# tool-recommender-bot/logparser

Measured on AMD Instinct MI355X. Metric: GB/s (and lines/s) of 'combined' log parsed per GPU and per 8xMI355X node, higher is better.
Workload: dtype u8

## Files before the change

logparser_amd/csrc/lp_device.h:

```cpp
#pragma once
#include <cstddef>
#include <type_traits>
#include <utility>

#include "lp_program.h"
#include "lp_fixed.h"

namespace lp {

enum : int { ST_OK = 0, ST_BAD = 1, ST_FALLBACK = 2,
             ST_REDO = 3,
             ST_REPAIR = 4 };

#if defined(LP_PROFILE) && defined(__HIP__)
static __device__ unsigned long long g_prof[PROF_WAVES * PROF_POINTS];
#endif
#if defined(LP_PROFILE) && defined(__HIP_DEVICE_COMPILE__)
__device__ __forceinline__ void lp_prof_mark(int k) {
    const unsigned long long t = clock64();
    const unsigned w = blockIdx.x - PROF_W0;
    const uint64_t act = __ballot(1);
    if (w < (unsigned)PROF_WAVES && (int)threadIdx.x % 64 == (int)__builtin_ctzll(act))
        __builtin_nontemporal_store(t, &g_prof[w * PROF_POINTS + k]);
}
// ... 2692 lines not shown

template <typename BP>
__host__ __device__ LP_INLINE bool utf8_ok(BP b, uint32_t n) {
    for (uint32_t i = 0; i < n;) {
        uint32_t c = b[i];
        if (c < 0x80) { ++i; continue; }
        int need;
        uint32_t cp;
        if (c >= 0xC2 && c <= 0xDF) { need = 1; cp = c & 0x1F; }
        else if (c >= 0xE0 && c <= 0xEF) { need = 2; cp = c & 0x0F; }
        else if (c >= 0xF0 && c <= 0xF4) { need = 3; cp = c & 0x07; }
        else return false;
        if (i + (uint32_t)need >= n) return false;
        for (int r = 1; r <= need; ++r) {
            if ((b[i + r] & 0xC0) != 0x80) return false;
            cp = (cp << 6) | (b[i + r] & 0x3F);
        }
        if (need == 2 && (cp < 0x800 || (cp >= 0xD800 && cp <= 0xDFFF))) return false;
        if (need == 3 && (cp < 0x10000 || cp > 0x10FFFF)) return false;
        i += need + 1;
    }
    return true;
}

template <typename LN>
__host__ __device__ LP_INLINE uint64_t decode_span(const LN& L, int a, int b, Arena& A) {
    uint32_t start = A.used;
    for (int q = a; q < b;) {
        uint32_t c = L[q];
        if (c == '%') { A.put(hexv(L[q + 1]) * 16 + hexv(L[q + 2])); q += 3; }
        else { A.put(c); ++q; }
    }
    if (!utf8_ok(A.p + start, A.used - start)) return ~0ull;
    return mkref(start, A.used - start, true);
}

__host__ __device__ LP_INLINE void put_encoded(Arena& A, uint32_t c) {
    const char* HX = "0123456789ABCDEF";
    A.put('%');
    A.put(HX[c >> 4]);
    A.put(HX[c & 15]);
}

__host__ __device__ LP_INLINE void store_word(LP_G uint8_t* p, uint32_t v) {
#if defined(__HIP_DEVICE_COMPILE__)
    *reinterpret_cast<LP_G uint32_t*>(p) = v;
#else
    __builtin_memcpy(p, &v, 4);
#endif
}
template <typename LN>
__host__ __device__ LP_INLINE uint64_t url_decode_value(const LN& L, int vs, int e, Arena& A) {
    const uint32_t st = A.used;
    uint32_t W = (L.o + (uint32_t)vs) >> 2;
    uint64_t ww = (uint64_t)L.word(W) | ((uint64_t)L.word_or0(W + 1) << 32);
    uint64_t acc = 0;
    uint32_t na = 0, out = st;
    for (int q = vs; q < e;) {
        while (na < 4 && q < e) {
            const uint32_t k = L.o + (uint32_t)q - 4 * W;
            const uint32_t c = (uint32_t)(ww >> (8 * k)) & 0xFFu;
            if (c == '%') {
                const uint32_t v =
                    hexv((uint32_t)(ww >> (8 * k + 8)) & 0xFFu) * 16 + hexv((uint32_t)(ww >> (8 * k + 16)) & 0xFFu);
                if (v < 0x80) { acc |= (uint64_t)v << (8 * na); na += 1; }
                else { acc |= (uint64_t)((0xC0 | (v >> 6)) | ((0x80 | (v & 0x3F)) << 8)) << (8 * na); na += 2; }
                q += 3;
            } else {
                acc |= (uint64_t)(c == '+' ? ' ' : c) << (8 * na);
                na += 1;
                ++q;
            }
            if (L.o + (uint32_t)q >= 4 * (W + 1)) {
                ++W;
                ww = (ww >> 32) | ((uint64_t)L.word_or0(W + 1) << 32);
            }
        }
        store_word(A.p + out, (uint32_t)acc);
        if (na >= 4) { out += 4; na -= 4; acc >>= 32; }
        else { out += na; na = 0; acc = 0; }
    }
    if (na) { store_word(A.p + out, (uint32_t)acc); out += na; }
    A.used = out;
    return mkref(st, A.used - st, true);
}

constexpr uint64_t REF_SKIP = ~0ull;

struct QueryTable {
    uint32_t tab = 0, reg = 0, count = 0, maxp = 0;
    int s = 0;
    int lp = -1;
    bool on = false, set = false;
    __host__ __device__ LP_INLINE void emit(LP_G uint8_t* region, int e) {
        if (e > s) {
            const uint64_t t0 = (uint64_t)(uint32_t)s | ((uint64_t)(uint32_t)e << 16) | ((uint64_t)(uint32_t)(lp + 1) << 48);
#if defined(__HIP_DEVICE_COMPILE__)
            typedef uint32_t u32x4_t __attribute__((ext_vector_type(4)));
            *reinterpret_cast<LP_G u32x4_t*>(region + tab + 16 * count) = u32x4_t{(uint32_t)t0, (uint32_t)(t0 >> 32), 0u, 0u};
#else
            LP_G uint64_t* t = (LP_G uint64_t*)(region + tab) + 2 * count;
            t[0] = t0;
            t[1] = 0;
#endif
            ++count;
        }
        lp = -1;
    }
};

template <typename LN>
__host__ __device__ LP_INLINE int piece_eq_rw(const LN& L, int s, int e, bool& rw) {
    rw = false;
    if (s >= e) return -1;
    const uint32_t A = L.o + (uint32_t)s, E = L.o + (uint32_t)e;
    uint32_t W = A >> 2;
    uint32_t valid = swar::HI << (8 * (A & 3));
    for (;;) {
        const uint32_t w = L.word(W);
        const uint32_t r = E - 4 * W;
        if (r < 4) valid &= swar::HI >> (8 * (4 - r));
        const uint32_t meq = swar::eq(w, '=') & valid;
        const uint32_t mrw = (swar::upper(w) | swar::needs_encode(w)) & valid;
        if (meq) {
            rw = rw || (mrw & ((meq & (0u - meq)) - 1u)) != 0;
            return (int)(4 * W + (uint32_t)swar::first(meq) - L.o);
        }
        rw = rw || mrw != 0;
        ++W;
        if (4 * W >= E) return -1;
        valid = swar::HI;
    }
}

struct QPrep {
    int s = 0, e = 0, eq = -1;
    bool rw = false, pv = false;
    uint32_t need = 0;
};
template <typename LN>
__host__ __device__ LP_INLINE QPrep query_prep(const LN& L, uint64_t t0) {
    QPrep q;
    q.s = (int)(t0 & 0xFFFFu);
    q.e = (int)((t0 >> 16) & 0xFFFFu);
    const int lp = (int)((t0 >> 48) & 0xFFFFu) - 1;
    q.eq = piece_eq_rw(L, q.s, q.e, q.rw);
    q.pv = q.eq >= 0 && lp > q.eq;
    const int ne = q.eq >= 0 ? q.eq : q.e;
    q.need = (q.rw ? (3u * (uint32_t)(ne - q.s) + 3u) & ~3u : 0u) + (q.pv ? ((uint32_t)(q.e - q.eq - 1) + 3u) & ~3u : 0u);
    return q;
}

template <typename LN>
__host__ __device__ LP_INLINE uint32_t query_finish(const Program& P, const QueryStage& Q, const LN& L, Arena& A,
                                                    const LP_G uint8_t* region, LP_G uint64_t* slot, const QPrep& qp) {
    const int s = qp.s, e = qp.e, eq = qp.eq;
    const int ne = eq >= 0 ? eq : e;
    const uint32_t a1 = A.used;
    uint64_t nref;
    if (qp.rw) {
        const char* HX = "0123456789abcdef";
        const uint32_t mark = A.used;
        for (int q = s; q < ne; ++q) {
            const uint32_t c = L[q];
            if (uri_needs_encode(c)) { A.put('%'); A.put(HX[c >> 4]); A.put(HX[c & 15]); }
            else A.put((c - 'A') < 26u ? (c | 32) : c);
        }
        nref = mkref(mark, A.used - mark, true);
        A.used = (A.used + 3) & ~3u;
    } else {
        nref = src_ref(L, s, ne - s);
    }
    bool want = Q.want_all;
    const uint32_t nlen = ref_len(nref);
    for (int k = 0; k < Q.n_names && !want; ++k) {
        if (Q.name_len[k] != nlen) continue;
        bool same = true;
        for (uint32_t q = 0; q < nlen && same; ++q) {
            const uint32_t c = qp.rw ? (uint32_t)region[ref_off(nref) + q] : L[s + (int)q];
            same = c == P.lit_byte((int)(Q.name_off[k] + q));
        }
        want = same;
    }
    if (!want) {
        slot[0] = REF_SKIP;
        slot[1] = 0;
        return A.used - a1;
    }
    uint64_t vref;
    if (eq < 0) vref = mkref(0, 0, false);
    else if (!qp.pv) vref = src_ref(L, eq + 1, e - eq - 1);
    else vref = url_decode_value(L, eq + 1, e, A);
    slot[0] = nref;
    slot[1] = vref;
    return A.used - a1;
}

template <typename LN>
__host__ __device__ LP_INLINE uint32_t query_piece(const Program& P, const QueryStage& Q, const LN& L, Arena& R,
                                                   LP_G uint64_t* slot) {
    const QPrep qp = query_prep(L, slot[0]);
    Arena A;
    if (!spill(R, qp.need, A)) {
        slot[0] = REF_SKIP;
        slot[1] = 0;
        return 0;
    }
    return query_finish(P, Q, L, A, R.p, slot, qp);
}

struct UriWalk {
    int fa = -1, h = -1, nh = 0, first_pct = -1;
    uint32_t rewr = 0;
    int resume = -1;
    QueryTable T;
};

template <typename LN>
__host__ __device__ LP_INLINE void uri_walk_fast(const Program& P, int u, const LN& L, int a, int b, uint32_t usep,
                                                 Arena& A, UriWalk& Wk) {
    const UriStage& U = P.uri[u];
    const int qsi = U.want_query ? U.query_stage : -1;
    QueryTable& T = Wk.T;
    int& fa = Wk.fa;
    int& first_pct = Wk.first_pct;
    uint32_t& rewr = Wk.rewr;
    int& resume = Wk.resume;
    LP_PROF(50 + 4 * u);
    for_uev_w(L, a, b, [&](int q, uint32_t w) {
        const uint32_t c = w & 0xFFu;
        if (c == '#' || c == ';' || c >= 0x80) { resume = q; return false; }
        if (c == '%') {
            if (q + 2 >= b || !is_hex((w >> 8) & 0xFFu) || !is_hex((w >> 16) & 0xFFu)) { resume = q; return false; }
            first_pct = first_pct < 0 ? q : first_pct;
            T.lp = q;
            return true;
        }
        if (c == '&' || c == '?') {
            rewr |= (c == '?' && fa >= 0) ? 2u : 0u;
            if (T.on) {
                T.emit(A.p, q);
                T.s = q + 1;
            } else if (fa < 0 && qsi >= 0) {
                T.on = T.set = true;
                T.maxp = usep + 1;
                T.tab = (A.used + 15) & ~15u;
                T.reg = T.tab + 16 * T.maxp;
                T.s = q + 1;
            }
            fa = fa < 0 ? q : fa;
            return true;
        }
        rewr |= (fa >= 0 && uri_needs_encode(c)) ? 2u : 0u;
        T.lp = c == '+' ? q : T.lp;
        return true;
    });
    LP_PROF(51 + 4 * u);
}

enum : int { UR_OFF = 0, UR_ON = 1, UR_DONE = 2 };
template <typename LN, typename Cols>
__host__ __device__ LP_INLINE int uri_repair(const Program& P, int u, const LN& L, int a, int b, Arena& R, Cols& C,
                                             int64_t li);

template <int MODE = UR_ON, typename LN, typename Cols, typename UO>
__host__ __device__ LP_INLINE int uri_stage_rest(const Program& P, int u, const LN& L, int a, int b, uint32_t usep,
                                                 Arena& A, Cols& C, int64_t li, UO& o, UriWalk& Wk,
                                                 int rfa = -1, bool noamp = false) {
    const UriStage& U = P.uri[u];
    const int qsi = U.want_query ? U.query_stage : -1;
    QueryTable& T = Wk.T;
    int& fa = Wk.fa;
    int& h = Wk.h;
    int& nh = Wk.nh;
    int& first_pct = Wk.first_pct;
    uint32_t& rewr = Wk.rewr;
    const int resume = Wk.resume;
    int st = ST_OK;
    if (resume >= 0) for_uev(L, resume, b, [&](int q, uint32_t c) {
        if (c >= 0x80) { st = ST_FALLBACK; return false; }
        if (c == '%') {
            if constexpr (MODE != UR_DONE)
                if (q + 2 >= b || !is_hex(L[q + 1]) || !is_hex(L[q + 2])) { st = ST_REPAIR; return false; }
            if (first_pct < 0) first_pct = q;
            rewr |= h >= 0 ? 1u : 0u;
            if (T.on && h < 0) T.lp = q;
        } else if (c == '#') {
            ++nh;
            if (T.on && h < 0) {
                T.emit(A.p, q);
                T.on = false;
            }
            if (h < 0) h = q;
            if constexpr (MODE != UR_DONE) {
                if (q + 1 < b) {
                    const uint32_t d = L[q + 1];
                    if (d == '&' || d == '?' || d == 'x') { st = ST_REPAIR; return false; }
                }
                if (q > a && L[q - 1] == '=') { st = ST_REPAIR; return false; }
            }
        } else if (c == ';') {
            if constexpr (MODE != UR_DONE) {
                int r = q - 1;
                while (r >= a && (is_alnum(L[r]) || L[r] == '#')) --r;
                if (r >= a && (L[r] == '&' || L[r] == '?')) { st = ST_REPAIR; return false; }
            }
        } else if ((c == '&' || c == '?')) {
            rewr |= (c == '?' && fa >= 0 && h < 0) ? 2u : 0u;
            if (T.on) {
                T.emit(A.p, q);
                T.s = q + 1;
            } else if (fa < 0 && h < 0 && qsi >= 0) {
                T.on = T.set = true;
                T.maxp = usep + 1;
                T.tab = (A.used + 15) & ~15u;
                T.reg = T.tab + 16 * T.maxp;
                T.s = q + 1;
            }
            if (fa < 0) fa = q;
            rewr |= h >= 0 ? 1u : 0u;
        } else {
            const bool enc = uri_needs_encode(c);
            rewr |= (fa >= 0 && h < 0 && enc) ? 2u : 0u;
            if (T.on && c == '+') T.lp = q;
        }
        return true;
    });
    LP_PROF(52 + 4 * u);
    bool fix = false;
    if constexpr (MODE == UR_ON) fix = st == ST_REPAIR;
    if (st != ST_OK && !fix) return st;
    if (!fix && T.set) {
        if (T.on) T.emit(A.p, b);
        A.used = T.reg;
        A.slack += 16 * (T.maxp - T.count);
        C.q_count[qsi][li] = T.count;
        C.q_params[qsi][li] = mkref(T.tab, 16 * T.count, true);
        o.qlist.set(qsi, T.tab);
        o.qpend.set(qsi, T.count);
    }
    LP_PROF(30 + 8 * u);
    if constexpr (MODE == UR_OFF) {
        if (nh > 1) return ST_REPAIR;
    } else if constexpr (MODE == UR_ON) {
        if (!fix && nh > 1) {
// ... 631 lines not shown
```

logparser_amd/csrc/uri.hip:

```cpp
#include "kernels_common.h"

namespace lp {

namespace {

constexpr uint32_t URI_CAP = 8512;
#ifndef LP_URI_QR
#define LP_URI_QR 4
#endif
#ifndef LP_URI_GR
#define LP_URI_GR 9
#endif

constexpr int OWNER_WORDS = LP_URI_GR;
constexpr int OWNER_LDS_WORDS = OWNER_WORDS + PW / 2;
struct OwnerRounds {
    uint64_t* hw;
    uint32_t* tab;
    uint32_t first;
    bool has;
    uint32_t b0;

    __device__ __forceinline__ OwnerRounds(uint64_t* words, uint32_t first_item, uint32_t cnt)
        : hw(words), tab(reinterpret_cast<uint32_t*>(words + OWNER_WORDS)), first(first_item), has(cnt != 0), b0(0) {
// ... 34 lines not shown
template <int NU>
__device__ __forceinline__ UriLane<NU> uri_lane(const Program& P, const Columns& C, int64_t li, bool active) {
    UriLane<NU> U;
    U.sp.fill(0);
    U.cs.fill(0);
    U.usep.fill(0);
    U.ok = false;
    U.fmt = 0;
    U.ls = 0;
    if (!active) return U;
    const uint8_t st = C.status[li];
    const int fmt = P.n_fmt > 1 ? (int)C.fmt_id[li] : 0;
    U.ls = C.line_off[li];
    const uint32_t tf = C.tok_flags[li];
    uint32_t raw[NU], kind[NU];
    for (int u = 0; u < NU; ++u) {
        raw[u] = 0;
        kind[u] = FL_FULL;
        if (u >= P.n_uri || P.uri[u].src_q >= 0) continue;
        if (P.uri[u].src_tok >= 0) {
            raw[u] = C.tok_span[P.uri[u].src_tok][li];
            kind[u] = (tf >> P.uri[u].src_tok) & 1u ? FL_NONE : FL_FULL;
        } else {
            raw[u] = C.fl_uri[P.uri[u].src_fl][li];
            kind[u] = C.fl_kind[P.uri[u].src_fl][li];
        }
    }
    U.ok = st == ST_OK;
    U.fmt = U.ok ? fmt : 0;
    if (U.ok)
        for (int u = 0; u < P.n_uri && u < NU; ++u) {
            const int a = (int)(raw[u] & 0xFFFF), b = (int)(raw[u] >> 16);
            if (P.uri[u].fmt == U.fmt && P.uri[u].src_q < 0 && kind[u] != FL_NONE && b > a) U.sp.set(u, mkspan(a, b));
        }
    return U;
}


template <bool SLOT, typename CL>
__device__ __forceinline__ void uri_walk_coop(const Program& P, int u, const CL& L, bool part, int a, int b,
                                              uint32_t usep, const Arena& A, uint64_t* heads, UriWalk& Wk) {
    const int lane = lane_id();
    const bool table = u >= 0 && P.uri[u].want_query && P.uri[u].query_stage >= 0;
    const uint32_t cnt = part ? usep : 0u;
    const uint32_t x = wave_incl_scan_dpp(cnt);
    const uint32_t eb = x - cnt, E = lane_value(x, 63);
    OwnerRounds OW(heads, eb, cnt);
    const uint32_t tab = (A.used + 15) & ~15u;
    const unsigned long long reg = (unsigned long long)(uintptr_t)A.p;
    int resume = -1, fa = -1, fpct = -1, lastB = -1, lastPP = -1;
    uint32_t count = 0;
    bool rw = false;
    for (uint32_t g0 = 0; g0 < E; g0 += PW) {
        const uint32_t g = g0 + (uint32_t)lane;
        const bool valid = g < E;
        OW.fill_at(g0);
        uint32_t ebo;
        const int ow = OW.owner(g0, ebo);
        const uint32_t oo = (uint32_t)__shfl((int)L.o, ow);
        const int oa = __shfl(a, ow), ob = __shfl(b, ow);
        uint32_t Aq = 0;
        if (valid) {
            const uint32_t A0 = oo + (uint32_t)oa, A1 = oo + (uint32_t)ob, WL = (A1 - 1) >> 6;
            uint32_t W = A0 >> 6, k = g - ebo;
            uint64_t m = L.mask(MC_UEV, W) & (~0ull << (A0 & 63));
            for (;;) {
                if (W == WL) m &= ~0ull >> (63 - ((A1 - 1) & 63));
                const uint32_t c = (uint32_t)__popcll(m);
                if (k < c || W >= WL) break;
                k -= c;
                ++W;
                m = L.mask(MC_UEV, W);
            }
            Aq = (W << 6) + select64(m, k);
        }
        const int q = (int)(Aq - oo);
        CL Lo = L;
        Lo.o = oo;
        Lo.n = ob;
        const uint32_t w = valid ? load_u32_at(Lo, q) : 0u;
        const uint32_t c = w & 0xFFu;
        const bool pct = c == '%';
        const bool bad_pct = pct && (q + 2 >= ob || !is_hex((w >> 8) & 0xFFu) || !is_hex((w >> 16) & 0xFFu));
        const bool stop = valid && (c == '#' || c == ';' || c >= 0x80 || bad_pct);
        const bool aq = c == '&' || c == '?';
        const int cres = __shfl(resume, ow), cfa = __shfl(fa, ow), clB = __shfl(lastB, ow), clPP = __shfl(lastPP, ow);
        const uint32_t ccount = (uint32_t)__shfl((int)count, ow);
        const int s0 = (int)ebo - (int)g0;
        const uint64_t below = (1ull << lane) - 1ull;
        const uint64_t seg_lt = valid ? below & (~0ull << (s0 > 0 ? s0 : 0)) : 0ull;
        const uint64_t Bstop = __ballot(stop);
        const bool live = valid && !stop && cres < 0 && !(Bstop & seg_lt);
        const uint64_t Baq = __ballot(live && aq);
        const uint64_t mfa = Baq & seg_lt;
        const int qfa = __shfl(q, mfa ? lsb64(mfa) : lane);
        const int fa_j = cfa >= 0 ? cfa : (mfa ? qfa : -1);
        const bool pp = live && ((pct && !bad_pct) || c == '+');
        const bool otable = SLOT ? __shfl((int)table, ow) != 0 : table;
        const bool isB = otable && live && aq && fa_j >= 0;
        const uint64_t BB = __ballot(isB), BPP = __ballot(pp);
        const uint64_t mB = BB & seg_lt, mP = BPP & seg_lt;
        const int qpb = __shfl(q, mB ? msb64(mB) : lane), qpp = __shfl(q, mP ? msb64(mP) : lane);
        const bool first_piece = !mB && clB < 0;
        const int pb = mB ? qpb : (clB >= 0 ? clB : fa_j);
        const int lpp = mP ? qpp : clPP;
        const int lp = first_piece ? lpp : (lpp > pb ? lpp : -1);
        const bool emit = isB && q > pb + 1;
        const uint64_t BE = __ballot(emit);
        const bool rwj = live && fa_j >= 0 && ((aq && c == '?') || (!aq && !pct && uri_needs_encode(c)));
        const uint64_t BR = __ballot(rwj);
        const unsigned long long oreg = __shfl(reg, ow);
        const uint32_t otab = (uint32_t)__shfl((int)tab, ow);
        if (emit) {
            const uint32_t idx = ccount + (uint32_t)__popcll(BE & seg_lt);
            const uint64_t t0 = (uint64_t)(uint32_t)(pb + 1) | ((uint64_t)(uint32_t)q << 16) | ((uint64_t)(uint32_t)(lp + 1) << 48);
            *reinterpret_cast<LP_G u32x4*>(reinterpret_cast<LP_G uint8_t*>(oreg) + otab + 16 * idx) =
                u32x4{(uint32_t)t0, (uint32_t)(t0 >> 32), 0u, 0u};
        }
        const int so = (int)eb - (int)g0, eo = (int)(eb + cnt) - (int)g0;
        const int so_c = so < 0 ? 0 : so > PW ? PW : so, eo_c = eo < 0 ? 0 : eo > PW ? PW : eo;
        const uint64_t segm = so_c < eo_c ? ((eo_c == PW ? ~0ull : (1ull << eo_c) - 1ull) & (~0ull << so_c)) : 0ull;
        const uint64_t ms = Bstop & segm, mf = Baq & segm, mpct = __ballot(live && pct) & segm, mb = BB & segm,
                       mpp = BPP & segm;
        const int q_s = __shfl(q, ms ? lsb64(ms) : lane), q_f = __shfl(q, mf ? lsb64(mf) : lane);
        const int q_p = __shfl(q, mpct ? lsb64(mpct) : lane), q_b = __shfl(q, mb ? msb64(mb) : lane);
        const int q_pp = __shfl(q, mpp ? msb64(mpp) : lane);
        if (resume < 0 && ms) resume = q_s;
        if (fa < 0 && mf) fa = q_f;
        if (fpct < 0 && mpct) fpct = q_p;
        if (mb) lastB = q_b;
        if (mpp) lastPP = q_pp;
        count += (uint32_t)__popcll(BE & segm);
        rw = rw || (BR & segm) != 0;
    }
    if (!part) return;
    Wk.resume = resume;
    Wk.fa = fa;
    Wk.first_pct = fpct;
    Wk.rewr = rw ? 2u : 0u;
    QueryTable& T = Wk.T;
    if (table && fa >= 0) {
        T.on = T.set = true;
        T.maxp = usep + 1;
        T.tab = tab;
        T.reg = tab + 16 * T.maxp;
        T.s = (lastB >= 0 ? lastB : fa) + 1;
        T.count = count;
        T.lp = lastB >= 0 ? (lastPP > lastB ? lastPP : -1) : lastPP;
    } else {
        T.lp = lastPP;
    }
}

template <int NU, int NQ, bool COOP, bool SLOT, bool QUEUE, typename LU, typename LL>
__device__ __forceinline__ void uri_wave(const Program& P, const Columns& C, UriLane<NU>& U, LU&& lu, LL&& ll,
                                         bool active, int64_t li, int64_t wave, uint64_t* heads, WaveCounts& WC,
                                         bool& redo) {
    const int lane = lane_id();
    const int nq = P.n_query < NQ ? P.n_query : NQ;
    uint32_t need = 0;
    if (U.ok)
        for (int u = 0; u < P.n_uri && u < NU; ++u) {
            const uint32_t s = U.sp.get(u);
            if (!s) continue;
            uint32_t ev;
            need += uri_need(P, u, lu(u), (int)(s & 0xFFFF), (int)(s >> 16), ev);
            U.usep.set(u, ev);
        }
    int lend = 0;
    if (U.ok) {
        for (int j = 0; j < P.n_list; ++j)
            if (P.list[j].fmt == U.fmt) lend = max(lend, (int)(C.tok_span[P.list[j].tok][li] >> 16));
        for (int j = 0; j < P.n_pair; ++j)
            if (P.pair[j].fmt == U.fmt) lend = max(lend, (int)(C.tok_span[P.pair[j].tok][li] >> 16));
    }
    if (lend) ll(lend, [&](const auto& LH) { need += list_need(P, U.fmt, LH, C, li) + pair_need(P, U.fmt, LH, C, li); });
    need = (need + 15) & ~15u;
    LP_PROF(29);
    const uint32_t x = wave_incl_scan_dpp(need);
    const uint32_t total = lane_value(x, 63);
    LP_PROF(20);
    const int shard = (int)(wave % ARENA_SHARDS);
    unsigned long long wbase = 0;
    if (lane == 63 && total) wbase = atomicAdd(&C.meta->shard_top[16 * shard], (unsigned long long)total + 12ull);
    wbase = (__shfl(wbase, 63) + 15) & ~15ull;
    const bool fits = wbase + total <= C.shard_cap;
    LP_PROF(26);
    uint32_t written = 0;
    unsigned long long my_region = 0;
    UriOutT<NQ> o;
    o.qlist.fill(0);
    o.qpend.fill(0);
    o.status = U.ok ? ST_OK : ST_BAD;
    Arena A{C.arena, 0, 0};
    bool live = false;
    if (U.ok) {
        if (!fits && need) {
            o.status = ST_FALLBACK;
            atomicAdd(&C.meta->arena_ovf, 1ull);
        } else {
            const unsigned long long mine = (unsigned long long)shard * C.shard_cap + wbase + x - need;
            my_region = mine;
            C.arena_base[li] = mine;
            A = Arena{C.arena + mine, 0, need};
            A.top = &C.meta->shard_top[16 * shard];
            A.base = wbase + x - need;
            A.limit = C.shard_cap;
            live = true;
        }
    }
    const int nu = P.n_uri < NU ? P.n_uri : NU;
    for (int sl = 0; sl < nu; ++sl) {
        int u = sl;
        if constexpr (SLOT) {
            u = -1;
            for (int v = 0, c = 0; v < nu; ++v)
                if (P.uri[v].fmt == U.fmt) {
                    if (c == sl) u = v;
                    ++c;
                }
            if (!__any(u >= 0)) break;
        }
        const bool fmt_ok = live && o.status == ST_OK && u >= 0 && P.uri[u].fmt == U.fmt;
        const uint32_t sp = U.sp.get(u);
        const int a = (int)(sp & 0xFFFF), b = (int)(sp >> 16);
        const bool part = fmt_ok && b > a;
        if (fmt_ok && !part) {
            C.u_flags[u][li] = 0;
            if (P.uri[u].query_stage >= 0) { C.q_count[P.uri[u].query_stage][li] = 0; C.q_params[P.uri[u].query_stage][li] = 0; }
        }
        LP_PROF(10 + 2 * sl);
        UriWalk Wk;
        if constexpr (COOP) {
            LP_PROF(50 + 4 * sl);
            uri_walk_coop<SLOT>(P, u, lu(u), part, a, b, U.usep.get(u), A, heads, Wk);
            LP_PROF(51 + 4 * sl);
        } else if (part) {
            uri_walk_fast(P, u, lu(u), a, b, U.usep.get(u), A, Wk);
        }
        if (part) {
            const int st = uri_stage_rest<UR_OFF>(P, u, lu(u), a, b, U.usep.get(u), A, C, li, o, Wk);
            if (st != ST_OK) o.status = st;
        }
        LP_PROF(11 + 2 * sl);
    }
    if (live && lend && o.status == ST_OK) {
        bool filled = true;
        ll(lend, [&](const auto& LH) { filled = list_fill(P, U.fmt, LH, A, C, li) && pair_fill(P, U.fmt, LH, A, C, li); });
        if (!filled) o.status = ST_FALLBACK;
    }
    if (live) {
        if (A.ovf) {
            o.status = ST_FALLBACK;
            atomicAdd(&C.meta->arena_ovf, 1ull);
        }
        written = A.used - A.slack + A.extra;
    }
    LP_PROF(21);
    if (nq > 0) {
        constexpr int QR = LP_URI_QR;
        __syncthreads();
        const bool has = U.ok && o.status == ST_OK && need != 0;
        const unsigned long long my_ab = has ? my_region : 0ull;
        uint64_t piece_ovf = 0;
        uint32_t np = 0;
        for (int qs = 0; qs < nq; ++qs) np += has ? o.qpend.get(qs) : 0u;
        const uint32_t incl = wave_incl_scan_dpp(np);
        const uint32_t base = incl - np, tot = lane_value(incl, 63);
        OwnerRounds OW(heads, base, np);
        auto piece = [&](int ow, uint32_t j, int& pq, uint32_t& soff) {
            uint32_t cum = 0;
            pq = 0;
            soff = 0;
            for (int qs = 0; qs < nq; ++qs) {
                const uint32_t c = (uint32_t)__shfl((int)(has ? o.qpend.get(qs) : 0u), ow);
                const uint32_t l = (uint32_t)__shfl((int)o.qlist.get(qs), ow);
                if (j >= cum && j < cum + c) {
                    pq = qs;
                    soff = l + 16 * (j - cum);
                }
                cum += c;
            }
        };
        auto owner_view = [&](int ow, int pq) {
            auto OL = owner_line(lu(P.query[0].uri), ow);
            for (int qs = 1; qs < nq; ++qs) {
                const auto V = owner_line(lu(P.query[qs].uri), ow);
                if (pq == qs) OL = V;
            }
            return OL;
        };
        for (uint32_t g0 = 0; g0 < tot; g0 += QR * PW) {
            int own[QR], pqs[QR];
            uint32_t soffs[QR];
            uint64_t t0[QR];
#pragma unroll
            for (int k = 0; k < QR; ++k) {
                own[k] = 0;
                pqs[k] = 0;
                soffs[k] = 0;
                t0[k] = 0;
                if (g0 + (uint32_t)(k * PW) >= tot) continue;
                const uint32_t g = g0 + (uint32_t)(k * PW + lane);
                OW.fill_at(g0 + (uint32_t)(k * PW));
                uint32_t ob;
                const int ow = OW.owner(g0 + (uint32_t)(k * PW), ob);
                own[k] = ow;
                const unsigned long long oab = __shfl(my_ab, ow);
                piece(ow, g - ob, pqs[k], soffs[k]);
                if (g < tot) t0[k] = *reinterpret_cast<const LP_G uint64_t*>(C.arena + oab + soffs[k]);
            }
            LP_PROF(17);
            QPrep qp[QR];
            uint32_t mine = 0;
#pragma unroll
            for (int k = 0; k < QR; ++k) {
                if (g0 + (uint32_t)(k * PW) >= tot) continue;
                const uint32_t g = g0 + (uint32_t)(k * PW + lane);
                const auto OL = owner_view(own[k], pqs[k]);
                if (g < tot) qp[k] = query_prep(OL, t0[k]);
                mine += qp[k].need;
            }
            LP_PROF(18);
            const uint32_t x = wave_incl_scan_dpp(mine);
            const uint32_t rtot = lane_value(x, 63);
            unsigned long long rbase = 0;
            if (lane == 63 && rtot) rbase = atomicAdd(&C.meta->shard_top[16 * shard], (unsigned long long)rtot);
            unsigned long long at = __shfl(rbase, 63) + x - mine;
            LP_PROF(19);
#pragma unroll
            for (int k = 0; k < QR; ++k) {
                if (g0 + (uint32_t)(k * PW) >= tot) continue;
                const uint32_t g = g0 + (uint32_t)(k * PW + lane);
                const int ow = own[k];
                const unsigned long long oab = __shfl(my_ab, ow);
                const auto OL = owner_view(ow, pqs[k]);
                bool povf = false;
                if (g < tot) {
                    LP_G uint64_t* slot = reinterpret_cast<LP_G uint64_t*>(C.arena + oab + soffs[k]);
                    const unsigned long long rel = oab - (unsigned long long)shard * C.shard_cap;
                    if (qp[k].need && (at + qp[k].need > C.shard_cap || at - rel + qp[k].need > 0x7FFFFFFFull)) {
                        slot[0] = REF_SKIP;
                        slot[1] = 0;
                        povf = true;
                        atomicAdd(&C.meta->arena_ovf, 1ull);
                    } else {
                        Arena A{C.arena + oab, (uint32_t)(at - rel), (uint32_t)(at - rel + qp[k].need)};
                        written += query_finish(P, P.query[pqs[k]], OL, A, C.arena + oab, slot, qp[k]);
                    }
                    at += qp[k].need;
                }
                for (uint64_t m = __ballot(povf); m; m &= m - 1) piece_ovf |= 1ull << __shfl(ow, (int)__builtin_ctzll(m));
            }
        }
        if (((piece_ovf >> lane) & 1) && o.status == ST_OK) o.status = ST_FALLBACK;
    }
    LP_PROF(22);
    redo = false;
    if (U.ok && o.status == ST_REPAIR) {
        o.status = ST_FALLBACK;
        if constexpr (QUEUE) {
            const unsigned long long k = atomicAdd(&C.meta->uri_fix_lines, 1ull);
            if (k < (unsigned long long)C.cap_lines) C.uri_fix_list[k] = (uint32_t)li;
        } else {
            redo = true;
        }
    }
    if (U.ok && o.status != ST_OK) C.status[li] = (uint8_t)o.status;
    for (int d = 32; d > 0; d >>= 1) written += __shfl_xor(written, d);
    const int st = !active ? -1 : U.ok ? o.status : (int)C.status[li];
    WC.act += (uint32_t)__popcll(__ballot(active));
    WC.ok += (uint32_t)__popcll(__ballot(st == ST_OK));
    WC.bad += (uint32_t)__popcll(__ballot(st == ST_BAD));
    WC.written += written;
}


template <int NU, int NQ, bool SLOT, uint32_t CAP>
__device__ __forceinline__ bool uri_compact(const uint8_t* __restrict__ buf, uint64_t nbytes, const Program& P,
                                            const Columns& C, int64_t wave, int64_t n_lines, uint32_t* cbuf,
                                            uint64_t* plane, uint64_t* heads, WaveCounts& WC, bool& redo) {
    const int lane = lane_id();
    const int64_t li = wave * PW + lane;
    const bool active = li < n_lines;
    LP_PROF(23);
    UriLane<NU> U = uri_lane<NU>(P, C, li, active);
    LP_PROF(27);
    uint64_t lo = ~0ull, hi = 0;
    for (int u = 0; u < P.n_uri && u < NU; ++u) {
        const uint32_t s = U.sp.get(u);
        if (!s) continue;
        lo = min(lo, U.ls + (s & 0xFFFF));
        hi = max(hi, U.ls + (s >> 16));
    }
    const uint64_t r0 = hi ? lo & ~15ull : 0;
    const uint32_t nb1 = hi ? (uint32_t)((((hi + 15) & ~15ull) - r0) >> 4) : 0u;
    const bool lists = P.n_list > 0 || P.n_pair > 0;
    uint64_t l0 = ~0ull, l1 = 0;
    if (lists && U.ok) {
        auto add = [&](int tok) {
            const uint32_t s = C.tok_span[tok][li];
            if ((s >> 16) > (s & 0xFFFFu)) {
                l0 = min(l0, U.ls + (s & 0xFFFFu));
                l1 = max(l1, U.ls + (s >> 16));
            }
        };
        for (int j = 0; j < P.n_list; ++j)
            if (P.list[j].fmt == U.fmt) add(P.list[j].tok);
        for (int j = 0; j < P.n_pair; ++j)
            if (P.pair[j].fmt == U.fmt) add(P.pair[j].tok);
    }
    const uint64_t q0 = l1 ? l0 & ~15ull : 0;
    const uint32_t nb2 = l1 ? (uint32_t)((((l1 + 15) & ~15ull) - q0) >> 4) : 0u;
    auto blocks = [&](uint32_t n, uint32_t& first) {
        const uint32_t x = wave_incl_scan_dpp(n);
        first = x - n;
        return lane_value(x, 63);
    };
    uint32_t cb, nb = nb1 + nb2;
    uint32_t tot = blocks(nb, cb);
    bool lin = lists;
    if (lists && 16 * tot + 16 > CAP) {
        lin = false;
        nb = nb1;
        tot = blocks(nb, cb);
    }
    if (16 * tot + 16 > CAP) return false;
    WC.gathered = 16 * tot;
    for (int u = 0; u < P.n_uri && u < NU; ++u) {
        const uint32_t s = U.sp.get(u);
        if (s) U.cs.set(u, 16 * cb + (uint32_t)(U.ls + (s & 0xFFFF) - r0));
    }
    constexpr int GR = LP_URI_GR;
    uint16_t* pl16 = reinterpret_cast<uint16_t*>(plane);
    OwnerRounds OW(heads, cb, nb);
    for (uint32_t g0 = 0; g0 < tot; g0 += GR * PW) {
        u32x4 v[GR];
        OW.fill(g0);
#pragma unroll
        for (int k = 0; k < GR; ++k) {
            v[k] = u32x4{0, 0, 0, 0};
            if (g0 + (uint32_t)(k * PW) >= tot) continue;
            const uint32_t g = g0 + (uint32_t)(k * PW + lane);
            uint32_t ocb;
            const int own = OW.owner(g0 + (uint32_t)(k * PW), ocb);
            const uint32_t j = g - ocb;
            uint64_t src = (uint64_t)__shfl((unsigned long long)r0, own) + 16ull * j;
            if (lin) {
                const uint32_t n1 = (uint32_t)__shfl(nb1, own);
                const uint64_t s1 = (uint64_t)__shfl((unsigned long long)q0, own);
                if (j >= n1) src = s1 + 16ull * (j - n1);
            }
            if (g < tot) v[k] = load16(buf, nbytes, src);
        }
        LP_PROF(28);
#pragma unroll
        for (int k = 0; k < GR; ++k) {
            const uint32_t g = g0 + (uint32_t)(k * PW + lane);
            if (g >= tot) continue;
            *reinterpret_cast<u32x4*>(cbuf + 4 * g) = v[k];
            pl16[g] = (uint16_t)bcls::classify16u(v[k][0], v[k][1], v[k][2], v[k][3]);
        }
    }
    LP_PROF(24);
    for (uint32_t g = tot + lane; g < ((tot + 1 + 3) & ~3u); g += PW) {
        *reinterpret_cast<u32x4*>(cbuf + 4 * g) = u32x4{0, 0, 0, 0};
        pl16[g] = 0;
    }
    __syncthreads();
    LP_PROF(25);
    typedef LineT<lds_bytes, lds_u64, 1> CL;
    auto lu = [&](int u) {
        const uint32_t s = U.sp.get(u);
        return CL{(lds_bytes)cbuf, U.cs.get(u) - (s & 0xFFFFu), (int)(s >> 16), (lds_u64)plane};
    };
    const LP_G uint8_t* lsp = (const LP_G uint8_t*)buf + U.ls;
    const uint32_t lmis = (uint32_t)((uintptr_t)lsp & 3);
    const uint32_t lorig = 16 * (cb + nb1) + (uint32_t)(U.ls - q0);
    auto ll = [&](int lend, auto&& f) {
        if (lin) f(LineT<lds_bytes>{(lds_bytes)cbuf, lorig, lend});
        else f(LineT<const LP_G uint8_t*>{lsp - lmis, lmis, lend});
    };
    uri_wave<NU, NQ, true, SLOT, CAP == URI_CAP>(P, C, U, lu, ll, active, li, wave, heads, WC, redo);
    return true;
}

#ifndef LP_URI_SLOT_WPE
#define LP_URI_SLOT_WPE 4
#endif
template <int NU, int NQ, bool SLOT>
__global__ __launch_bounds__(PW, SLOT ? LP_URI_SLOT_WPE : 4) void k_uri_lines(const uint8_t* __restrict__ buf, uint64_t nbytes,
                                                     const DeviceArgs* __restrict__ args) {
    const Program& P = args->prog;
    const Columns& C = args->cols;
    const int64_t n_lines = (int64_t)C.meta->n_lines;
    const int64_t wave = blockIdx.x;
    if (wave * PW >= n_lines || C.meta->cap_ovf) return;
    __shared__ __attribute__((aligned(16))) uint32_t cbuf[URI_CAP / 4 + 16];
    __shared__ uint64_t plane[URI_CAP / 64 + 1];
    __shared__ uint64_t heads[OWNER_LDS_WORDS];
    WaveCounts WC;
    bool redo;
    if (uri_compact<NU, NQ, SLOT, URI_CAP>(buf, nbytes, P, C, wave, n_lines, cbuf, plane, heads, WC, redo)) WC.store(C, wave);
    else if (lane_id() == 0) C.uri_ovf_list[atomicAdd(&C.meta->uri_ovf_waves, 1ull)] = (uint32_t)wave;
}

__device__ __forceinline__ void uri_redo_line(const uint8_t* __restrict__ buf, uint64_t nbytes, const Program& P,
                                              const Columns& C, int64_t n_lines, int64_t li) {
    if ((uint64_t)li >= (uint64_t)n_lines) return;
    const uint64_t s = C.line_off[li], e = C.line_off[li + 1] - 1;
    if (e < s || e - s > 0xFFFFull || e > nbytes) return;
    const int n = crlf_len((int)(e - s), e > s ? buf[e - 1] : 0u);
    const LP_G uint8_t* ls = (const LP_G uint8_t*)(buf) + s;
    const uint32_t mis = (uint32_t)((uintptr_t)ls & 3);
    const LineT<const LP_G uint8_t*> L{ls - mis, mis, n};
    const int fmt = P.n_fmt > 1 ? (int)C.fmt_id[li] : 0;
    RegArr<MAX_URI> sp, usep;
    sp.fill(0);
    usep.fill(0);
    uint32_t need = 0;
    for (int u = 0; u < P.n_uri; ++u) {
        int a, b;
        if (P.uri[u].fmt != fmt || !uri_source_cols(P, C, li, u, a, b) || b > n) continue;
        uint32_t ev;
        need += uri_need(P, u, L, a, b, ev);
        sp.set(u, mkspan((uint32_t)a, (uint32_t)b));
        usep.set(u, ev);
    }
    need += list_need(P, fmt, L, C, li) + pair_need(P, fmt, L, C, li);
    need = (need + 15) & ~15u;
    const int shard = (int)((li / PW) % ARENA_SHARDS);
    LP_G unsigned long long* top = &C.meta->shard_top[16 * shard];
    const unsigned long long x = (atomicAdd(top, (unsigned long long)need + 12ull) + 15) & ~15ull;
    int st = ST_FALLBACK;
    uint32_t written = 0;
    if (x + need > C.shard_cap) {
        atomicAdd(&C.meta->arena_ovf, 1ull);
    } else {
        const unsigned long long mine = (unsigned long long)shard * C.shard_cap + x;
        C.arena_base[li] = mine;
        Arena A{C.arena + mine, 0, need};
        A.top = top;
        A.base = x;
        A.limit = C.shard_cap;
        UriOut o;
        o.qlist.fill(0);
        o.qpend.fill(0);
        auto lu = [&](int) { return L; };
        phase2<UR_ON>(P, fmt, lu, sp, usep, o, A, C, li);
        if (o.status == ST_OK) query_pieces_serial(P, lu, o, A);
        if (o.status == ST_OK && (!list_fill(P, fmt, L, A, C, li) || !pair_fill(P, fmt, L, A, C, li))) o.status = ST_FALLBACK;
        if (A.ovf) {
            o.status = ST_FALLBACK;
            atomicAdd(&C.meta->arena_ovf, 1ull);
        }
        st = o.status;
        written = A.used - A.slack + A.extra;
    }
    LP_G uint32_t* wc = C.wave_counts + WC_WORDS * (size_t)(li / PW);
    if (st != ST_FALLBACK) {
        C.status[li] = (uint8_t)st;
        atomicAdd(&wc[st == ST_OK ? 1 : 2], 1u);
        atomicSub(&wc[3], 1u);
    }
    if (written) atomicAdd(&wc[4], written);
}

constexpr uint32_t URI_CAP_OVF = 4 * URI_CAP;
template <int NU, int NQ, bool SLOT>
__global__ __launch_bounds__(PW) void k_uri_overflow(const uint8_t* __restrict__ buf, uint64_t nbytes,
                                                     const DeviceArgs* __restrict__ args) {
    const Program& P = args->prog;
    const Columns& C = args->cols;
    const int64_t n_lines = (int64_t)C.meta->n_lines;
    const uint64_t nq = C.meta->uri_ovf_waves;
    const uint64_t nfix = min((uint64_t)(uint32_t)C.meta->uri_fix_lines, (uint64_t)C.cap_lines);
    __shared__ __attribute__((aligned(16))) uint32_t cbuf[URI_CAP_OVF / 4 + 16];
    __shared__ uint64_t plane[URI_CAP_OVF / 64 + 1];
    __shared__ uint64_t heads[OWNER_LDS_WORDS];
    for (uint64_t q = blockIdx.x; q < nq; q += gridDim.x) {
        const int64_t wave = C.uri_ovf_list[q];
        WaveCounts WC;
        bool redo = false;
        if (!uri_compact<NU, NQ, SLOT, URI_CAP_OVF>(buf, nbytes, P, C, wave, n_lines, cbuf, plane, heads, WC, redo)) {
            const WaveLines W = wave_lines(C, wave, n_lines, nbytes);
            UriLane<NU> U = uri_lane<NU>(P, C, W.li, W.active);
            const LP_G uint8_t* ls = (const LP_G uint8_t*)(buf) + W.s;
            const uint32_t mis = (uint32_t)((uintptr_t)ls & 3);
            const LineT<const LP_G uint8_t*> L{ls - mis, mis, crlf_len_hbm(buf, W)};
            auto lu = [&](int) { return L; };
            auto ll = [&](int lend, auto&& f) { f(LineT<const LP_G uint8_t*>{ls - mis, mis, lend}); };
            uri_wave<NU, NQ, false, SLOT, false>(P, C, U, lu, ll, W.active, W.li, wave, heads, WC, redo);
        }
        __syncthreads();
        WC.store(C, wave);
        if (__any(redo)) {
            __threadfence();
            if (redo) {
                atomicAdd(&C.meta->uri_fix_lines, 1ull << 32);
                uri_redo_line(buf, nbytes, P, C, n_lines, wave * PW + lane_id());
            }
        }
    }
    for (uint64_t q = (uint64_t)blockIdx.x * PW + (uint64_t)lane_id(); q < nfix; q += (uint64_t)gridDim.x * PW)
        uri_redo_line(buf, nbytes, P, C, n_lines, (int64_t)C.uri_fix_list[q]);
}

__global__ __launch_bounds__(PW) void k_derived_lines(const uint8_t* __restrict__ buf, uint64_t nbytes,
                                                      const DeviceArgs* __restrict__ args) {
    const Program& P = args->prog;
    const Columns& C = args->cols;
    const int64_t n_lines = (int64_t)C.meta->n_lines;
    const int64_t wave = blockIdx.x;
    if (wave * PW >= n_lines || C.meta->cap_ovf) return;
    const WaveLines W = wave_lines(C, wave, n_lines, nbytes);
    int st = W.active ? (int)C.status[W.li] : -1;
    if (st == ST_OK) {
        const int fmt = P.n_fmt > 1 ? (int)C.fmt_id[W.li] : 0;
        const LP_G uint8_t* ls = (const LP_G uint8_t*)(buf) + W.s;
        const uint32_t mis = (uint32_t)((uintptr_t)ls & 3);
        const unsigned long long ab = C.arena_base[W.li];
        const int shard = (int)(ab / C.shard_cap);
        Arena R{C.arena + ab, 0, 0};
        R.top = &C.meta->shard_top[16 * shard];
        R.base = ab - (unsigned long long)shard * C.shard_cap;
        R.limit = C.shard_cap;
        st = derived_line(P, fmt, ls - mis, mis, crlf_len_hbm(buf, W), R, C, W.li);
        if (R.ovf) atomicAdd(&C.meta->arena_ovf, 1ull);
        if (st != ST_OK) C.status[W.li] = (uint8_t)st;
    }
    const uint32_t ok = (uint32_t)__popcll(__ballot(st == ST_OK)), bad = (uint32_t)__popcll(__ballot(st == ST_BAD));
    if (lane_id() == 0) {
        LP_G uint32_t* wc = C.wave_counts + WC_WORDS * (size_t)wave;
        const uint32_t act = wc[0];
        wc[1] = ok;
        wc[2] = bad;
        wc[3] = act - ok - bad;
    }
}

}

int launch_uri(const ParseLaunch& a, const DeviceArgs* d_args, hipStream_t s) {
    const int64_t waves = parse_waves(a.cap_lines);
    if (waves == 0 || !a.uri) return 0;
    const int64_t grid = waves < 1024 ? waves : 1024;
    if (!a.chunked) {
        hipLaunchKernelGGL((k_uri_lines<MAX_URI, MAX_QUERY, true>), dim3((unsigned)waves), dim3(PW), 0, s, a.buf,
                           a.nbytes, d_args);
        hipLaunchKernelGGL((k_uri_overflow<MAX_URI, MAX_QUERY, true>), dim3((unsigned)grid), dim3(PW), 0, s, a.buf,
                           a.nbytes, d_args);
    } else if (a.n_uri <= 2 && a.n_query <= 2) {
        hipLaunchKernelGGL((k_uri_lines<2, 2, false>), dim3((unsigned)waves), dim3(PW), 0, s, a.buf, a.nbytes, d_args);
        hipLaunchKernelGGL((k_uri_overflow<2, 2, false>), dim3((unsigned)grid), dim3(PW), 0, s, a.buf, a.nbytes, d_args);
    } else {
        hipLaunchKernelGGL((k_uri_lines<MAX_URI, MAX_QUERY, false>), dim3((unsigned)waves), dim3(PW), 0, s, a.buf,
                           a.nbytes, d_args);
        hipLaunchKernelGGL((k_uri_overflow<MAX_URI, MAX_QUERY, false>), dim3((unsigned)grid), dim3(PW), 0, s, a.buf,
                           a.nbytes, d_args);
    }
    if (a.derived) hipLaunchKernelGGL(k_derived_lines, dim3((unsigned)waves), dim3(PW), 0, s, a.buf, a.nbytes, d_args);
    return hipGetLastError() == hipSuccess ? 0 : -1;
}

#if defined(LP_PROFILE)
int prof_read_uri(unsigned long long* out) {
    return hipMemcpyFromSymbol(out, HIP_SYMBOL(g_prof), sizeof(unsigned long long) * PROF_WAVES * PROF_POINTS) == hipSuccess ? 0 : -1;
}
int prof_clear_uri() {
    static unsigned long long z[PROF_WAVES * PROF_POINTS];
    return hipMemcpyToSymbol(HIP_SYMBOL(g_prof), z, sizeof z) == hipSuccess ? 0 : -1;
}
#endif

}
```

Measured before the change: 685.3.

## Defer percent-decoding of query values into a compacted wave-wide batch

```diff
diff --git a/logparser_amd/csrc/lp_device.h b/logparser_amd/csrc/lp_device.h
--- a/logparser_amd/csrc/lp_device.h
+++ b/logparser_amd/csrc/lp_device.h
@@ -2868,12 +2868,10 @@
 }
 
 template <typename LN>
-__host__ __device__ LP_INLINE uint32_t query_finish(const Program& P, const QueryStage& Q, const LN& L, Arena& A,
-                                                    const LP_G uint8_t* region, LP_G uint64_t* slot, const QPrep& qp) {
+__host__ __device__ LP_INLINE bool query_name(const Program& P, const QueryStage& Q, const LN& L, Arena& A,
+                                              const LP_G uint8_t* region, const QPrep& qp, uint64_t& nref) {
     const int s = qp.s, e = qp.e, eq = qp.eq;
     const int ne = eq >= 0 ? eq : e;
-    const uint32_t a1 = A.used;
-    uint64_t nref;
     if (qp.rw) {
         const char* HX = "0123456789abcdef";
         const uint32_t mark = A.used;
@@ -2898,15 +2896,24 @@
         }
         want = same;
     }
-    if (!want) {
+    return want;
+}
+template <typename LN>
+__host__ __device__ LP_INLINE uint64_t query_value_plain(const LN& L, const QPrep& qp) {
+    if (qp.eq < 0) return mkref(0, 0, false);
+    return src_ref(L, qp.eq + 1, qp.e - qp.eq - 1);
+}
+template <typename LN>
+__host__ __device__ LP_INLINE uint32_t query_finish(const Program& P, const QueryStage& Q, const LN& L, Arena& A,
+                                                    const LP_G uint8_t* region, LP_G uint64_t* slot, const QPrep& qp) {
+    const uint32_t a1 = A.used;
+    uint64_t nref;
+    if (!query_name(P, Q, L, A, region, qp, nref)) {
         slot[0] = REF_SKIP;
         slot[1] = 0;
         return A.used - a1;
     }
-    uint64_t vref;
-    if (eq < 0) vref = mkref(0, 0, false);
-    else if (!qp.pv) vref = src_ref(L, eq + 1, e - eq - 1);
-    else vref = url_decode_value(L, eq + 1, e, A);
+    const uint64_t vref = qp.pv ? url_decode_value(L, qp.eq + 1, qp.e, A) : query_value_plain(L, qp);
     slot[0] = nref;
     slot[1] = vref;
     return A.used - a1;
diff --git a/logparser_amd/csrc/uri.hip b/logparser_amd/csrc/uri.hip
--- a/logparser_amd/csrc/uri.hip
+++ b/logparser_amd/csrc/uri.hip
@@ -210,10 +210,55 @@
     }
 }
 
+constexpr int URI_CAPD = PW;
+constexpr uint32_t QDESC_NONE = ~0u;
+template <typename LN>
+struct QDescs {
+    static constexpr int WORDS = LN::has_masks ? 2 : 4;
+    uint64_t* buf;
+    __device__ __forceinline__ void post(uint32_t d, const LN& OL, int vs, int e, uint32_t used, uint32_t reg,
+                                         uint32_t soff) const {
+        const uint32_t S = OL.o + (uint32_t)vs, E = OL.o + (uint32_t)e;
+        u32x4* q = reinterpret_cast<u32x4*>(buf + WORDS * d);
+        if constexpr (LN::has_masks) {
+            q[0] = u32x4{S | E << 16, used, reg, soff};
+        } else {
+            const unsigned long long b = (unsigned long long)(uintptr_t)OL.b;
+            q[0] = u32x4{S, E, reg, soff};
+            q[1] = u32x4{(uint32_t)b, (uint32_t)(b >> 32), used, 0u};
+        }
+    }
+    __device__ __forceinline__ void post_none(uint32_t d) const {
+        *reinterpret_cast<u32x4*>(buf + WORDS * d) = u32x4{0u, 0u, 0u, QDESC_NONE};
+    }
+    __device__ __forceinline__ bool take(uint32_t d, const LN& L0, LN& V, int& S, int& E, uint32_t& used, uint32_t& reg,
+                                         uint32_t& soff) const {
+        const u32x4* q = reinterpret_cast<const u32x4*>(buf + WORDS * d);
+        const u32x4 a = q[0];
+        V = L0;
+        V.o = 0;
+        reg = a[2];
+        soff = a[3];
+        if constexpr (LN::has_masks) {
+            S = (int)(a[0] & 0xFFFFu);
+            E = (int)(a[0] >> 16);
+            used = a[1];
+        } else {
+            const u32x4 c = q[1];
+            V.b = reinterpret_cast<decltype(V.b)>((uintptr_t)((unsigned long long)c[0] | (unsigned long long)c[1] << 32));
+            S = (int)a[0];
+            E = (int)a[1];
+            used = c[2];
+        }
+        V.n = E;
+        return soff != QDESC_NONE;
+    }
+};
+
 template <int NU, int NQ, bool COOP, bool SLOT, bool QUEUE, typename LU, typename LL>
 __device__ __forceinline__ void uri_wave(const Program& P, const Columns& C, UriLane<NU>& U, LU&& lu, LL&& ll,
-                                         bool active, int64_t li, int64_t wave, uint64_t* heads, WaveCounts& WC,
-                                         bool& redo) {
+                                         bool active, int64_t li, int64_t wave, uint64_t* heads, uint64_t* scratch,
+                                         WaveCounts& WC, bool& redo) {
     const int lane = lane_id();
     const int nq = P.n_query < NQ ? P.n_query : NQ;
     uint32_t need = 0;
@@ -241,7 +286,7 @@
     const int shard = (int)(wave % ARENA_SHARDS);
     unsigned long long wbase = 0;
     if (lane == 63 && total) wbase = atomicAdd(&C.meta->shard_top[16 * shard], (unsigned long long)total + 12ull);
-    wbase = (__shfl(wbase, 63) + 15) & ~15ull;
+    wbase = (((unsigned long long)lane_value((uint32_t)wbase, 63) | (unsigned long long)lane_value((uint32_t)(wbase >> 32), 63) << 32) + 15) & ~15ull;
     const bool fits = wbase + total <= C.shard_cap;
     LP_PROF(26);
     uint32_t written = 0;
@@ -348,6 +393,26 @@
             }
             return OL;
         };
+        typedef decltype(lu(0)) QL;
+        const QDescs<QL> QD{scratch};
+        const unsigned long long w0 = (unsigned long long)shard * C.shard_cap + wbase;
+        LP_G uint8_t* const wreg = C.arena + w0;
+        auto decode_waiting = [&](uint32_t n) {
+            LP_PT_DECL
+            __syncthreads();
+            if ((uint32_t)lane < n) {
+                QL V;
+                int S, E;
+                uint32_t used, reg, soff;
+                if (QD.take((uint32_t)lane, lu(P.query[0].uri), V, S, E, used, reg, soff)) {
+                    Arena A{wreg + reg, used, used};
+                    reinterpret_cast<LP_G uint64_t*>(wreg + reg + soff)[1] = url_decode_value(V, S, E, A);
+                    written += A.used - used;
+                }
+            }
+            __syncthreads();
+            LP_PACC(57);
+        };
         for (uint32_t g0 = 0; g0 < tot; g0 += QR * PW) {
             int own[QR], pqs[QR];
             uint32_t soffs[QR];
@@ -386,10 +451,20 @@
             if (lane == 63 && rtot) rbase = atomicAdd(&C.meta->shard_top[16 * shard], (unsigned long long)rtot);
             unsigned long long at = __shfl(rbase, 63) + x - mine;
             LP_PROF(19);
+            uint32_t nwait = 0;
 #pragma unroll
             for (int k = 0; k < QR; ++k) {
                 if (g0 + (uint32_t)(k * PW) >= tot) continue;
                 const uint32_t g = g0 + (uint32_t)(k * PW + lane);
+                const bool pv = g < tot && qp[k].pv;
+                const uint64_t PB = __ballot(pv);
+                const uint32_t nb = (uint32_t)__popcll(PB);
+                if (nwait + nb > (uint32_t)URI_CAPD) {
+                    decode_waiting(nwait);
+                    nwait = 0;
+                }
+                const uint32_t d = nwait + __builtin_amdgcn_mbcnt_hi((uint32_t)(PB >> 32), __builtin_amdgcn_mbcnt_lo((uint32_t)PB, 0u));
+                nwait += nb;
                 const int ow = own[k];
                 const unsigned long long oab = __shfl(my_ab, ow);
                 const auto OL = owner_view(ow, pqs[k]);
@@ -401,15 +476,28 @@
                         slot[0] = REF_SKIP;
                         slot[1] = 0;
                         povf = true;
+                        if (pv) QD.post_none(d);
                         atomicAdd(&C.meta->arena_ovf, 1ull);
                     } else {
                         Arena A{C.arena + oab, (uint32_t)(at - rel), (uint32_t)(at - rel + qp[k].need)};
-                        written += query_finish(P, P.query[pqs[k]], OL, A, C.arena + oab, slot, qp[k]);
+                        const uint32_t a1 = A.used;
+                        uint64_t nref;
+                        const bool want = query_name(P, P.query[pqs[k]], OL, A, C.arena + oab, qp[k], nref);
+                        if (!want) {
+                            slot[0] = REF_SKIP;
+                            slot[1] = 0;
+                        } else {
+                            slot[0] = nref;
+                            if (!pv) slot[1] = query_value_plain(OL, qp[k]);
+                        }
+                        if (pv) QD.post(d, OL, qp[k].eq + 1, qp[k].e, A.used, (uint32_t)(oab - w0), want ? soffs[k] : QDESC_NONE);
+                        written += A.used - a1;
                     }
                     at += qp[k].need;
                 }
                 for (uint64_t m = __ballot(povf); m; m &= m - 1) piece_ovf |= 1ull << __shfl(ow, (int)__builtin_ctzll(m));
             }
+            if (nwait) decode_waiting(nwait);
         }
         if (((piece_ovf >> lane) & 1) && o.status == ST_OK) o.status = ST_FALLBACK;
     }
@@ -539,7 +627,7 @@
         if (lin) f(LineT<lds_bytes>{(lds_bytes)cbuf, lorig, lend});
         else f(LineT<const LP_G uint8_t*>{lsp - lmis, lmis, lend});
     };
-    uri_wave<NU, NQ, true, SLOT, CAP == URI_CAP>(P, C, U, lu, ll, active, li, wave, heads, WC, redo);
+    uri_wave<NU, NQ, true, SLOT, CAP == URI_CAP>(P, C, U, lu, ll, active, li, wave, heads, plane, WC, redo);
     return true;
 }
 
@@ -555,7 +643,8 @@
     const int64_t wave = blockIdx.x;
     if (wave * PW >= n_lines || C.meta->cap_ovf) return;
     __shared__ __attribute__((aligned(16))) uint32_t cbuf[URI_CAP / 4 + 16];
-    __shared__ uint64_t plane[URI_CAP / 64 + 1];
+    __shared__ __attribute__((aligned(16))) uint64_t plane[URI_CAP / 64 + 1];
+    static_assert(sizeof(plane) >= URI_CAPD * 16, "the plane holds URI_CAPD descriptors of the compact view");
     __shared__ uint64_t heads[OWNER_LDS_WORDS];
     WaveCounts WC;
     bool redo;
@@ -634,7 +723,8 @@
     const uint64_t nq = C.meta->uri_ovf_waves;
     const uint64_t nfix = min((uint64_t)(uint32_t)C.meta->uri_fix_lines, (uint64_t)C.cap_lines);
     __shared__ __attribute__((aligned(16))) uint32_t cbuf[URI_CAP_OVF / 4 + 16];
-    __shared__ uint64_t plane[URI_CAP_OVF / 64 + 1];
+    __shared__ __attribute__((aligned(16))) uint64_t plane[URI_CAP_OVF / 64 + 1];
+    static_assert(sizeof(plane) >= URI_CAPD * 32 && URI_CAP_OVF + 64 <= 0xFFFF, "URI_CAPD descriptors of either view; 16-bit offsets");
     __shared__ uint64_t heads[OWNER_LDS_WORDS];
     for (uint64_t q = blockIdx.x; q < nq; q += gridDim.x) {
         const int64_t wave = C.uri_ovf_list[q];
@@ -648,7 +738,7 @@
             const LineT<const LP_G uint8_t*> L{ls - mis, mis, crlf_len_hbm(buf, W)};
             auto lu = [&](int) { return L; };
             auto ll = [&](int lend, auto&& f) { f(LineT<const LP_G uint8_t*>{ls - mis, mis, lend}); };
-            uri_wave<NU, NQ, false, SLOT, false>(P, C, U, lu, ll, W.active, W.li, wave, heads, WC, redo);
+            uri_wave<NU, NQ, false, SLOT, false>(P, C, U, lu, ll, W.active, W.li, wave, heads, plane, WC, redo);
         }
         __syncthreads();
         WC.store(C, wave);
```

Measured after the change: 701.7 (median of 6 runs). 2.4% higher.
